# dnjulek/vapoursynth-zip

Measured on AMD Instinct MI355X. Metric: frames/sec at 4K YUV420P16: Bilateral, BoxBlur, SSIMULACRA2 on 1/2/4/8 MI355X, higher is better.
Workload: dtype u16; 1 GPU; vszip.BoxBlur hradius=vradius=13, 3840x2160 YUV420P16, splitmix64 noise, HBM-resident; parallelism=frame-parallel x1, arena_candidates=20

## Files before the change

### vapoursynth-zip_amd/csrc/boxblur_ct.hpp

```cpp
#pragma once
#include <cmath>
#include <cstdlib>
#include <utility>

#include "common.hpp"

namespace {

#ifndef VSZIP_ST_AUX
#define VSZIP_ST_AUX 2
#endif
#ifndef VSZIP_LD_AUX
#define VSZIP_LD_AUX 0
#endif
#ifndef VSZIP_ST8_AUX
#define VSZIP_ST8_AUX 0
#endif
#ifndef VSZIP_ST16_AUX
#define VSZIP_ST16_AUX 2
#endif
constexpr int kStoreAux = VSZIP_ST_AUX, kLoadAux = VSZIP_LD_AUX, kStoreAux8 = VSZIP_ST8_AUX, kStoreAux16 = VSZIP_ST16_AUX;
typedef uint32_t U32x4 __attribute__((ext_vector_type(4)));
typedef uint32_t U32x2 __attribute__((ext_vector_type(2)));

constexpr int kMaxPlanes = 48;
constexpr int PX = 8;

struct BBPlane {
    const void *src;
    void *dst;
    int sstride, dstride;
    int w, h;
    int block0;
    int ntx;
    int nbands;
    int nperiods;
    int cx0;
};

struct BBParams {
    BBPlane p[kMaxPlanes];
    int nplanes;
    int band_rows;
    int nblocks;
};

constexpr int kRingMaxPlanes = 192;
constexpr int kRingMaxBlocks = 8192;
struct RingParams {
    BBPlane p[kRingMaxPlanes];
    int nplanes;
    int nblocks;
    uint8_t plane_of_block[kRingMaxBlocks];
};

__device__ __forceinline__ int ct_tap_row(int k, int i, int radius, int ih) {
    const int dist_from_bottom = ih - 1 - i;
    if (k < radius) return (i < radius - k) ? min(radius - k - i, ih - 1) : (i - radius + k);
    return (dist_from_bottom < k - radius) ? (i - min(k - radius - dist_from_bottom, i)) : (i - radius + k);
}

template <typename T>
struct Raw8;
template <>
struct Raw8<uint16_t> {
    uint4 q;
};
template <>
struct Raw8<uint8_t> {
    uint2 q;
};

__device__ __forceinline__ void unpack8(const Raw8<uint16_t> &r, uint32_t v[PX]) {
    v[0] = r.q.x & 0xffffu; v[1] = r.q.x >> 16;
    v[2] = r.q.y & 0xffffu; v[3] = r.q.y >> 16;
    v[4] = r.q.z & 0xffffu; v[5] = r.q.z >> 16;
    v[6] = r.q.w & 0xffffu; v[7] = r.q.w >> 16;
}

__device__ __forceinline__ void unpack8(const Raw8<uint8_t> &r, uint32_t v[PX]) {
    v[0] = r.q.x & 0xffu; v[1] = (r.q.x >> 8) & 0xffu; v[2] = (r.q.x >> 16) & 0xffu; v[3] = r.q.x >> 24;
    v[4] = r.q.y & 0xffu; v[5] = (r.q.y >> 8) & 0xffu; v[6] = (r.q.y >> 16) & 0xffu; v[7] = r.q.y >> 24;
}

__device__ __forceinline__ void pack8(const uint32_t v[PX], Raw8<uint16_t> &r) {
    r.q.x = v[0] | (v[1] << 16);
    r.q.y = v[2] | (v[3] << 16);
    r.q.z = v[4] | (v[5] << 16);
    r.q.w = v[6] | (v[7] << 16);
}

__device__ __forceinline__ void pack8(const uint32_t v[PX], Raw8<uint8_t> &r) {
    r.q.x = v[0] | (v[1] << 8) | (v[2] << 16) | (v[3] << 24);
    r.q.y = v[4] | (v[5] << 8) | (v[6] << 16) | (v[7] << 24);
}

template <typename T, int PXN>
struct RawN : Raw8<T> {};
template <>
struct RawN<uint8_t, 16> {
    uint4 q;
};
template <typename T>
__device__ __forceinline__ void unpackN(const RawN<T, 8> &r, uint32_t v[8]) {
    unpack8(static_cast<const Raw8<T> &>(r), v);
}
__device__ __forceinline__ void unpackN(const RawN<uint8_t, 16> &r, uint32_t v[16]) {
    const uint32_t dw[4] = {r.q.x, r.q.y, r.q.z, r.q.w};
#pragma unroll
    for (int k = 0; k < 16; ++k) v[k] = (dw[k >> 2] >> (8 * (k & 3))) & 0xffu;
}

__device__ __forceinline__ int mirror_col(int c, int w) {
    c = c < 0 ? -c - 1 : c;
    c = c >= w ? 2 * w - 1 - c : c;
    return min(max(c, 0), w - 1);
}

template <typename T>
__device__ __forceinline__ Raw8<T> load8(const T *row, int vx0, int w, bool fast) {
    Raw8<T> r;
    if (fast) {
        r.q = *reinterpret_cast<const decltype(r.q) *>(row + vx0);
    } else {
        uint32_t v[PX];
#pragma unroll
        for (int k = 0; k < PX; ++k) v[k] = row[mirror_col(vx0 + k, w)];
        pack8(v, r);
    }
    return r;
}

template <typename T>
__device__ __forceinline__ void store8(T *row, int x0, int w, bool fast, const uint32_t o[PX]);

template <>
__device__ __forceinline__ void store8<uint16_t>(uint16_t *row, int x0, int w, bool fast, const uint32_t o[PX]) {
    if (fast) {
        uint4 q;
        q.x = (o[0] & 0xffffu) | (o[1] << 16);
        q.y = (o[2] & 0xffffu) | (o[3] << 16);
        q.z = (o[4] & 0xffffu) | (o[5] << 16);
        q.w = (o[6] & 0xffffu) | (o[7] << 16);
        *reinterpret_cast<uint4 *>(row + x0) = q;
    } else {
#pragma unroll
        for (int k = 0; k < PX; ++k)
            if (x0 + k < w) row[x0 + k] = (uint16_t)o[k];
    }
}

template <>
__device__ __forceinline__ void store8<uint8_t>(uint8_t *row, int x0, int w, bool fast, const uint32_t o[PX]) {
    if (fast) {
        uint2 q;
        q.x = (o[0] & 0xffu) | ((o[1] & 0xffu) << 8) | ((o[2] & 0xffu) << 16) | (o[3] << 24);
        q.y = (o[4] & 0xffu) | ((o[5] & 0xffu) << 8) | ((o[6] & 0xffu) << 16) | (o[7] << 24);
        *reinterpret_cast<uint2 *>(row + x0) = q;
    } else {
#pragma unroll
        for (int k = 0; k < PX; ++k)
            if (x0 + k < w) row[x0 + k] = (uint8_t)o[k];
    }
}

template <int R>
struct CtGeom {
    static constexpr int K = 2 * R + 1;
    static constexpr int NE = (R + 1 + PX - 1) / PX;
    static constexpr int HL = NE * PX;
    static constexpr int HR = ((R + PX - 1) / PX) * PX;
    static constexpr int OUT_LANES = 64 - NE - HL / PX - HR / PX;
    static constexpr int TWO = OUT_LANES * PX;
};

__device__ __forceinline__ void wave_lds_fence() {
    __builtin_amdgcn_fence(__ATOMIC_RELEASE, "wavefront");
    __builtin_amdgcn_wave_barrier();
    __builtin_amdgcn_fence(__ATOMIC_ACQUIRE, "wavefront");
}

template <typename T, int R, bool DPP>
__global__ __launch_bounds__(64) void boxblur_ct_int_kernel(const BBParams prm) {
    using G = CtGeom<R>;
    constexpr uint32_t K = G::K;
    constexpr uint32_t MAGIC = (uint32_t)(((1ull << 32) + K - 1) / K);
    constexpr uint64_t INV = ((1ull << 32) + R) / K;
    constexpr uint32_t INV2 = (uint32_t)(INV >> 16);
    constexpr uint32_t INVLO = (uint32_t)(INV & 0xffffu);

    __shared__ __attribute__((aligned(16))) uint32_t P[64 * PX];

    int pi = 0;
    const int b = blockIdx.x;
#pragma unroll 1
    for (int i = 1; i < prm.nplanes; ++i)
        if (b >= prm.p[i].block0) pi = i;
    const BBPlane pl = prm.p[pi];
    const int lb = b - pl.block0;
    const int tx = lb % pl.ntx;
    const int by = lb / pl.ntx;
    const int w = pl.w, h = pl.h;
    const int y0 = by * prm.band_rows;
    const int y1 = min(y0 + prm.band_rows, h);
    const T *src = static_cast<const T *>(pl.src);
    T *dst = static_cast<T *>(pl.dst);

    const int lane = threadIdx.x;
    const int X0 = tx * G::TWO;
    const int vx0 = lane < G::NE ? lane * PX : X0 - G::HL + (lane - G::NE) * PX;
    constexpr int VB = sizeof(T) * PX;
    const bool src_al = ((reinterpret_cast<uintptr_t>(src) | (uintptr_t)((size_t)pl.sstride * sizeof(T))) & (VB - 1)) == 0;
    const bool dst_al = ((reinterpret_cast<uintptr_t>(dst) | (uintptr_t)((size_t)pl.dstride * sizeof(T))) & (VB - 1)) == 0;
    const bool in_fast = src_al && vx0 >= 0 && vx0 + PX <= w;
    const bool is_out = lane >= G::NE + G::HL / PX && lane < G::NE + G::HL / PX + G::OUT_LANES && vx0 < w;
    const bool out_fast = dst_al && vx0 + PX <= w;

    uint32_t col[PX];
#pragma unroll
    for (int k = 0; k < PX; ++k) col[k] = 0;
#pragma unroll 1
    for (int k = 0; k < (int)K; ++k) {
        uint32_t v[PX];
        unpack8(load8<T>(src + (size_t)ct_tap_row(k, y0, R, h) * pl.sstride, vx0, w, in_fast), v);
#pragma unroll
        for (int j = 0; j < PX; ++j) col[j] += v[j];
    }

    const int ci = lane * PX;
#pragma unroll 1
    for (int i = y0; i < y1; ++i) {
        Raw8<T> an, sn;
        const bool more = i + 1 < y1;
        if (more) {
            const int n = i + 1;
            const int ar = (n + R < h) ? n + R : n - 1;
            const int sr = (n <= R) ? R - n + 1 : n - R - 1;
            an = load8<T>(src + (size_t)ar * pl.sstride, vx0, w, in_fast);
            sn = load8<T>(src + (size_t)sr * pl.sstride, vx0, w, in_fast);
        }

        uint32_t p[PX];
#pragma unroll
        for (int k = 0; k < PX; ++k) p[k] = __umulhi(col[k] + R, MAGIC);
#pragma unroll
        for (int k = 1; k < PX; ++k) p[k] += p[k - 1];
        const uint32_t incl = DPP ? wave_incl_scan_dpp(p[PX - 1]) : wave_incl_scan_shfl(p[PX - 1]);
        const uint32_t base = incl - p[PX - 1];
#pragma unroll
        for (int k = 0; k < PX; ++k) p[k] += base;
        *reinterpret_cast<uint4 *>(&P[ci]) = make_uint4(p[0], p[1], p[2], p[3]);
        *reinterpret_cast<uint4 *>(&P[ci + 4]) = make_uint4(p[4], p[5], p[6], p[7]);
        wave_lds_fence();

        if (is_out) {
            const uint32_t e0 = P[R] + P[R - 1];
            const uint32_t krow = 32768u + (uint32_t)(((uint64_t)e0 * INVLO) >> 16);
            uint32_t o[PX];
#pragma unroll
            for (int k = 0; k < PX; ++k) {
                const uint32_t e = P[ci + k + R] - P[ci + k - R - 1];
                o[k] = (uint32_t)(((uint64_t)e * INV2 + krow) >> 16);
            }
            store8<T>(dst + (size_t)i * pl.dstride, vx0, w, out_fast, o);
        }
        wave_lds_fence();

        if (more) {
            uint32_t a[PX], sb[PX];
            unpack8(an, a);
            unpack8(sn, sb);
#pragma unroll
            for (int k = 0; k < PX; ++k) col[k] += a[k] - sb[k];
        }
    }
}



template <int R, int SLOT_VGPRS = 4, int PXN = 8, int RV = R>
struct RingGeom {
    static constexpr int K = 2 * RV + 1;
    static constexpr int HL = ((R + 1 + PXN - 1) / PXN) * PXN;
    static constexpr int HR = ((R + PXN - 1) / PXN) * PXN;
#ifdef VSZIP_RING_OUT_LANES
    static constexpr int OUT_LANES = VSZIP_RING_OUT_LANES < 64 - HL / PXN - HR / PXN ? VSZIP_RING_OUT_LANES : 64 - HL / PXN - HR / PXN;
#else
    static constexpr int OUT_LANES = 64 - HL / PXN - HR / PXN;
#endif
    static constexpr int TWO = OUT_LANES * PXN;
    static constexpr int est_vgprs(int d) { return (2 * RV + 1 + d) * SLOT_VGPRS + (PXN == 16 ? 104 : 56); }
    static constexpr int tier(int v) { return v <= 128 ? 4 : (v <= 168 ? 3 : 2); }
    static constexpr int D3 = (2 * RV + 4) % 3 == 0 ? 3 : ((2 * RV + 6) % 3 == 0 ? 5 : 7);
#ifdef VSZIP_RING_D
    static constexpr int D = VSZIP_RING_D | 1;
    static constexpr int KL = (2 * RV + 1 + D) % 3 == 0 ? 3 : 2;
#else
    static constexpr bool SHALLOW = tier(est_vgprs(1)) > tier(est_vgprs(D3));
    static constexpr int D = SHALLOW ? 1 : D3;
    static constexpr int KL = SHALLOW ? 2 : 3;
#endif
    static constexpr int NR = 2 * RV + 1 + D;
#ifdef VSZIP_RING_WPE
    static constexpr int WPE = VSZIP_RING_WPE;
#else
    static constexpr int WPE = (SLOT_VGPRS == 2 && PXN == 8) ? (tier(est_vgprs(D)) > 3 ? 3 : tier(est_vgprs(D))) : tier(est_vgprs(D));
#endif
    static_assert(NR % KL == 0, "K-column ring must divide the period");
    static constexpr uint32_t MAGIC = K > 1 ? (uint32_t)(((1ull << 32) + K - 1) / K) : 0u;
};

template <typename T, int R, bool GENERAL, int PXN = 8, bool HONLY = false>
struct RingWave {
    static_assert(PXN == 8 || (PXN == 16 && sizeof(T) == 1 && !GENERAL), "16 pixels a lane: 8-bit planes, whole 16-pixel groups");
    static constexpr int RV = HONLY ? 0 : R;
    using G = RingGeom<R, (int)(sizeof(T) * PXN / 4), PXN, RV>;
    using RawT = RawN<T, PXN>;
    using Vec = decltype(RawT{}.q);
    static constexpr int NR = G::NR;
    static constexpr uint64_t INV = ((1ull << 32) + R) / (uint64_t)(2 * R + 1);
    static constexpr uint32_t INV2 = (uint32_t)(INV >> 16);

    RawT ring[NR];
    uint32_t col[PXN];
    uint32_t kcol;
    uint32_t kwgt;
    uint32_t kvo;
    uint32_t kn[G::KL], ko[G::KL];
    uint32_t kn_off, ko_off;
    uint32_t kr_prev;
    uint32_t *P;
    const char *srcb;
    char *dstb;
    uint32_t coff;
    uint32_t doff;
    uint32_t next_off;
    uint32_t out_off;
    uint32_t srow, drow;
    int w, h, lane, c0;
    bool rev, ld_ok, is_out, out_full;
    bool plain;
    __amdgpu_buffer_rsrc_t rs, rd;
    uint32_t sdoff;
    uint32_t psel;
    static constexpr uint32_t kOOB = 0xfffffff0u;

    __device__ __forceinline__ RawT fetch_off(uint32_t row_off) const {
        RawT t;
        if constexpr (sizeof(T) * PXN == 16) {
            const auto v = __builtin_amdgcn_raw_buffer_load_b128(rs, coff, row_off, sizeof(T) == 2 ? kLoadAux : 0);
            t.q = make_uint4(v[0], v[1], v[2], v[3]);
        } else {
            const auto v = __builtin_amdgcn_raw_buffer_load_b64(rs, coff, row_off, 0);
            t.q = make_uint2(v[0], v[1]);
        }
        return t;
    }
    __device__ __forceinline__ uint32_t fetch_px(uint32_t row_off) const {
        if constexpr (sizeof(T) == 2)
            return __builtin_amdgcn_raw_buffer_load_b16(rs, kvo, row_off, 0);
        else
            return __builtin_amdgcn_raw_buffer_load_b8(rs, kvo, row_off, 0);
    }
    __device__ __forceinline__ uint32_t krow_now() const {
        constexpr uint32_t INVLO = (uint32_t)(INV & 0xffffu);
        uint32_t v = __umul24(G::K > 1 ? __umulhi(kcol, G::MAGIC) : kcol, kwgt);
        v += (uint32_t)__builtin_amdgcn_update_dpp(0, (int)v, 0x111, 0xf, 0xf, false);
        v += (uint32_t)__builtin_amdgcn_update_dpp(0, (int)v, 0x112, 0xf, 0xf, false);
        v += (uint32_t)__builtin_amdgcn_update_dpp(0, (int)v, 0x114, 0xf, 0xf, false);
        v += (uint32_t)__builtin_amdgcn_update_dpp(0, (int)v, 0x118, 0xf, 0xf, false);
        uint32_t e0;
        if constexpr (R < 16) {
            e0 = (uint32_t)__builtin_amdgcn_readlane((int)v, 15);
        } else {
            v += (uint32_t)__builtin_amdgcn_update_dpp(0, (int)v, 0x142, 0xa, 0xf, false);
            e0 = (uint32_t)__builtin_amdgcn_readlane((int)v, 31);
        }
        return 32768u + (uint32_t)(((uint64_t)e0 * INVLO) >> 16);
    }

    __device__ __forceinline__ void fix_order(RawT &r) const {
        if constexpr (GENERAL) return;
        if constexpr (sizeof(T) * PXN == 16) {
            const uint4 o = r.q;
            r.q.x = __builtin_amdgcn_perm(o.w, o.x, psel);
            r.q.y = __builtin_amdgcn_perm(o.z, o.y, psel);
            r.q.z = __builtin_amdgcn_perm(o.y, o.z, psel);
            r.q.w = __builtin_amdgcn_perm(o.x, o.w, psel);
        } else {
            const uint2 o = r.q;
            r.q.x = __builtin_amdgcn_perm(o.y, o.x, psel);
            r.q.y = __builtin_amdgcn_perm(o.x, o.y, psel);
        }
    }
    __device__ __forceinline__ uint32_t row_off(int v) const {
        const int r = v < 0 ? -v : (v < h ? v : v - RV - 1);
        return (uint32_t)min(r, h - 1) * srow;
    }

    template <int J>
    __device__ __forceinline__ void fill(int y0) {
        ring[J] = fetch_off(row_off(y0 - RV + J));
    }
    template <int J>
    __device__ __forceinline__ void accum() {
        uint32_t v[PXN];
        fix_order(ring[J]);
        unpackN(ring[J], v);
#pragma unroll
        for (int k = 0; k < PXN; ++k) col[k] += v[k];
    }
    template <int... J>
    __device__ __forceinline__ void fill_all(int y0, std::integer_sequence<int, J...>) {
        (fill<(J + G::K) % NR>(y0), ...);
    }
    template <int... J>
    __device__ __forceinline__ void accum_all(std::integer_sequence<int, J...>) {
        (accum<J>(), ...);
    }

    static __device__ __forceinline__ int pidx(int c) { return (c & (PXN - 1)) * 64 + c / PXN; }

    __device__ __forceinline__ void window_sums(const uint32_t *Pb, uint32_t e[PXN]) const {
        if constexpr (!GENERAL) {
#pragma unroll
            for (int k = 0; k < PXN; ++k) {
                const int hi = k + R, lo = k - R - 1;
                const int hi_px = hi & (PXN - 1), hi_ln = hi / PXN;
                const int lo_px = lo & (PXN - 1), lo_ln = (lo - lo_px) / PXN;
                e[k] = Pb[hi_px * 64 + lane + hi_ln] - Pb[lo_px * 64 + lane + lo_ln];
            }
        } else {
            const int off = lane * PXN - c0;
            auto lds = [&](int idx) { return Pb[pidx(min(max(idx, 0), 64 * PXN - 1))]; };
            const uint32_t qw = lds(w - 1 + off);
#pragma unroll
            for (int k = 0; k < PXN; ++k) {
                const int x = c0 + k;
                const int lo = x - R - 1, ml = R - x - 1;
                uint32_t v = lds(min(x + R, w - 1) + off) + qw - lds(min(2 * w - 2 - x - R, w - 1) + off);
                v -= lo >= 0 ? lds(lo + off) : 0u;
                v += ml >= 0 ? lds(ml + off) : 0u;
                e[k] = v;
            }
        }
    }

    __device__ __forceinline__ void emit_row(const uint32_t e[PXN], uint32_t row_off_bytes, uint32_t kr, bool live) const {
        if constexpr (GENERAL) {
            if (!live || !is_out) return;
        }
        uint32_t t[PXN];
#pragma unroll
        for (int k = 0; k < PXN; ++k) t[k] = __umul24(e[k], INV2) + kr;
        if constexpr (!GENERAL) {
#ifdef VSZIP_DIAG_NO_STORE
            const uint32_t vo = (live && lane == 8) ? sdoff : kOOB;
#else
            const uint32_t vo = live ? sdoff : kOOB;
#endif
            if constexpr (sizeof(T) == 2) {
                U32x4 v;
                v.x = __builtin_amdgcn_perm(t[1], t[0], 0x07060302u);
                v.y = __builtin_amdgcn_perm(t[3], t[2], 0x07060302u);
                v.z = __builtin_amdgcn_perm(t[5], t[4], 0x07060302u);
                v.w = __builtin_amdgcn_perm(t[7], t[6], 0x07060302u);
                __builtin_amdgcn_raw_buffer_store_b128(v, rd, vo, row_off_bytes, kStoreAux);
            } else if constexpr (PXN == 16) {
                uint32_t dw[4];
#pragma unroll
                for (int g = 0; g < 4; ++g) {
                    const uint32_t a0 = __builtin_amdgcn_perm(t[4 * g + 1], t[4 * g], 0x0c0c0602u);
                    const uint32_t a1 = __builtin_amdgcn_perm(t[4 * g + 3], t[4 * g + 2], 0x0c0c0602u);
                    dw[g] = a0 | (a1 << 16);
                }
                U32x4 v;
                v.x = dw[0];
                v.y = dw[1];
                v.z = dw[2];
                v.w = dw[3];
                __builtin_amdgcn_raw_buffer_store_b128(v, rd, vo, row_off_bytes, kStoreAux16);
            } else {
                U32x2 v;
                const uint32_t a0 = __builtin_amdgcn_perm(t[1], t[0], 0x0c0c0602u);
                const uint32_t a1 = __builtin_amdgcn_perm(t[3], t[2], 0x0c0c0602u);
                const uint32_t a2 = __builtin_amdgcn_perm(t[5], t[4], 0x0c0c0602u);
                const uint32_t a3 = __builtin_amdgcn_perm(t[7], t[6], 0x0c0c0602u);
                v.x = a0 | (a1 << 16);
                v.y = a2 | (a3 << 16);
                __builtin_amdgcn_raw_buffer_store_b64(v, rd, vo, row_off_bytes, kStoreAux8);
            }
        } else {
            T *q = reinterpret_cast<T *>(dstb + (row_off_bytes + doff));
            if (out_full) {
                if constexpr (sizeof(T) == 2) {
                    uint4 v;
                    v.x = __builtin_amdgcn_perm(t[1], t[0], 0x07060302u);
                    v.y = __builtin_amdgcn_perm(t[3], t[2], 0x07060302u);
                    v.z = __builtin_amdgcn_perm(t[5], t[4], 0x07060302u);
                    v.w = __builtin_amdgcn_perm(t[7], t[6], 0x07060302u);
                    *reinterpret_cast<uint4 *>(q) = v;
                } else {
                    uint2 v;
                    const uint32_t a0 = __builtin_amdgcn_perm(t[1], t[0], 0x0c0c0602u);
                    const uint32_t a1 = __builtin_amdgcn_perm(t[3], t[2], 0x0c0c0602u);
                    const uint32_t a2 = __builtin_amdgcn_perm(t[5], t[4], 0x0c0c0602u);
                    const uint32_t a3 = __builtin_amdgcn_perm(t[7], t[6], 0x0c0c0602u);
                    v.x = a0 | (a1 << 16);
                    v.y = a2 | (a3 << 16);
                    *reinterpret_cast<uint2 *>(q) = v;
                }
            } else {
#pragma unroll
                for (int k = 0; k < PXN; ++k)
                    if (c0 + k < w) q[k] = (T)(t[k] >> 16);
            }
        }
    }

    template <int S>
    __device__ __forceinline__ void step(int i, int y0) {
        uint32_t *Pa = P + (S & 1) * (64 * PXN);
        const uint32_t *Pb = P + ((S & 1) ^ 1) * (64 * PXN);
        __builtin_amdgcn_sched_barrier(0);

        uint32_t e[PXN];
        const bool have_prev = S > 0 || i > y0;
#ifdef VSZIP_DIAG_NO_HORIZONTAL
#pragma unroll
        for (int k = 0; k < PXN; ++k) e[k] = col[k];
#else
        if (!GENERAL || have_prev) window_sums(Pb, e);
#endif

        uint32_t p[PXN];
#pragma unroll
        for (int k = 0; k < PXN; ++k) {
            if constexpr (G::K == 1) {
                p[k] = col[k];
            } else if constexpr (sizeof(T) == 1) {
                constexpr uint32_t M19 = (uint32_t)(((1u << 19) + G::K - 1) / G::K);
                static_assert((uint64_t)(255u * G::K + RV) * (M19 * G::K - (1u << 19)) < (1u << 19), "8-bit divide-by-k shortcut must be exact");
                p[k] = __umul24(col[k], M19) >> 19;
            } else {
                p[k] = __umulhi(col[k], G::MAGIC);
            }
        }
        if constexpr (GENERAL) {
            const uint32_t m = ld_ok ? 0xffffffffu : 0u;
#pragma unroll
            for (int k = 0; k < PXN; ++k) p[k] &= m;
        }
#ifdef VSZIP_DIAG_NO_HORIZONTAL
        (void)Pa;
        kr_prev += p[0] + p[7];
#else
#pragma unroll
        for (int k = 1; k < PXN; ++k) p[k] += p[k - 1];
        const uint32_t incl = wave_incl_scan_dpp(p[PXN - 1]);
        const uint32_t base = incl - p[PXN - 1];
#pragma unroll
        for (int k = 0; k < PXN; ++k) Pa[k * 64 + lane] = p[k] + base;
#endif

        {
            constexpr int E = (S + 1 + 2 * RV) % NR;
            uint32_t a[PXN], sb[PXN];
            fix_order(ring[E]);
            unpackN(ring[E], a);
            unpackN(ring[S], sb);
#pragma unroll
            for (int k = 0; k < PXN; ++k) col[k] += a[k] - sb[k];
#ifdef VSZIP_DIAG_NO_LOAD
            if (next_off == 0xffffffffu) ring[S] = fetch_off(next_off);
#else
            ring[S] = fetch_off(next_off);
#endif

        }
        const uint32_t kr_cur = krow_now();
        {
            constexpr int J = S % G::KL;
            kcol += kn[J] - ko[J];
#ifndef VSZIP_DIAG_NO_KCOL
            kn[J] = fetch_px(kn_off);
            ko[J] = fetch_px(ko_off);
#endif

        }

        emit_row(e, out_off, kr_prev, have_prev);
        out_off += have_prev ? drow : 0u;
        kr_prev = kr_cur;
        if (plain) {
            next_off += srow;
            kn_off += srow;
            ko_off += srow;
        } else {
            next_off = row_off(i + 2 + RV + G::D);
            kn_off = row_off(i + 2 + RV + G::KL);
            ko_off = row_off(i + 1 - RV + G::KL);
        }
#ifndef VSZIP_DIAG_NO_FENCE
        wave_lds_fence();
#endif
    }

    template <int... S>
    __device__ __forceinline__ void period(int i0, int y0, std::integer_sequence<int, S...>) {
        (step<S>(i0 + S, y0), ...);
    }
};

template <typename T, int R, bool GENERAL, int PXN = 8, bool HONLY = false>
__global__ __launch_bounds__(64, (GENERAL ? 2 : RingGeom<R, (int)(sizeof(T) * PXN / 4), PXN, (HONLY ? 0 : R)>::WPE)) void boxblur_ct_ring_kernel(const RingParams prm) {
    using W = RingWave<T, R, GENERAL, PXN, HONLY>;
    using G = typename W::G;
    constexpr int RV = W::RV;
    static_assert(G::NR % 2 == 0 && G::NR <= 64, "ring period must be even and fit a wave");
    __shared__ __attribute__((aligned(16))) uint32_t P[2 * 64 * PXN];

    const int chunk = (prm.nblocks + 7) >> 3;
    const int b = (int)(blockIdx.x & 7) * chunk + (int)(blockIdx.x >> 3);
    if (b >= prm.nblocks) return;
    const int pi = prm.plane_of_block[b];
    const BBPlane pl = prm.p[pi];
    const int lb = b - pl.block0;
    const int tx = lb % pl.ntx;
    const int by = lb / pl.ntx;
    const int p0 = (int)((long)by * pl.nperiods / pl.nbands);
    const int p1 = (int)((long)(by + 1) * pl.nperiods / pl.nbands);
    const int band_rows = (p1 - p0) * G::NR;
    const int y0 = min(p0 * G::NR, pl.h - band_rows);
    const int w = pl.w;

    W st;
    st.P = P;
    st.w = w;
    st.h = pl.h;
    st.srow = (uint32_t)pl.sstride * (uint32_t)sizeof(T);
    st.drow = (uint32_t)pl.dstride * (uint32_t)sizeof(T);
    st.srcb = static_cast<const char *>(pl.src);
    st.dstb = static_cast<char *>(pl.dst);
    const int lane = threadIdx.x;
    st.lane = lane;
    const int vc0 = pl.cx0 + tx * G::TWO - G::HL + lane * PXN;
    st.c0 = vc0;
    st.is_out = lane >= G::HL / PXN && lane < G::HL / PXN + G::OUT_LANES && vc0 < w;
    st.doff = (uint32_t)(max(vc0, 0) * (int)sizeof(T));
    st.out_full = vc0 + PXN <= w;
    if constexpr (!GENERAL) {
        int g = vc0;
        st.rev = false;
        if (vc0 < 0) {
            g = -vc0 - PXN;
            st.rev = true;
        } else if (vc0 >= w) {
            g = 2 * w - vc0 - PXN;
            st.rev = true;
        }
        g = min(max(g, 0), w - PXN);
        st.coff = (uint32_t)(g * (int)sizeof(T));
        st.ld_ok = true;
    } else {
        st.rev = false;
        st.ld_ok = vc0 >= 0 && vc0 < w;
        st.coff = (uint32_t)(min(max(vc0, 0), ((w - 1) / PXN) * PXN) * (int)sizeof(T));
    }

    st.psel = st.rev ? (sizeof(T) == 2 ? 0x05040706u : 0x04050607u) : 0x03020100u;
    st.sdoff = st.is_out ? st.doff : W::kOOB;
    st.rs = __builtin_amdgcn_make_buffer_rsrc(const_cast<void *>(pl.src), 0, (int)((uint32_t)pl.h * st.srow), 0x00020000);
    st.rd = __builtin_amdgcn_make_buffer_rsrc(pl.dst, 0, (int)((uint32_t)pl.h * st.drow), 0x00020000);
    st.plain = (y0 - RV >= 0) && (y0 + band_rows + RV + G::D + 2 < pl.h);

    st.fill_all(y0, std::make_integer_sequence<int, G::NR>{});
#pragma unroll
    for (int k = 0; k < PXN; ++k) st.col[k] = RV;
    st.accum_all(std::make_integer_sequence<int, (int)G::K>{});
    {
        const int kc = min(lane, R);
        st.kvo = (uint32_t)(kc * (int)sizeof(T));
        st.kwgt = lane < R ? 2u : (lane == R ? 1u : 0u);
        uint32_t acc = RV;
#pragma unroll
        for (int k = 0; k < (int)G::K; ++k) acc += st.fetch_px(st.row_off(y0 - RV + k));
        st.kcol = acc;
#pragma unroll
        for (int j = 0; j < G::KL; ++j) {
            st.kn[j] = st.fetch_px(st.row_off(y0 + j + 1 + RV));
            st.ko[j] = st.fetch_px(st.row_off(y0 + j - RV));
        }
        st.kn_off = st.row_off(y0 + G::KL + 1 + RV);
        st.ko_off = st.row_off(y0 + G::KL - RV);
        st.kr_prev = 0;
    }
    st.next_off = st.row_off(y0 + 1 + RV + G::D);
    st.out_off = (uint32_t)y0 * st.drow;

    const int y1 = y0 + band_rows;
#pragma unroll 1
    for (int i0 = y0; i0 < y1; i0 += G::NR) st.period(i0, y0, std::make_integer_sequence<int, G::NR>{});
    {
        uint32_t e[PXN];
        st.window_sums(P + 64 * PXN, e);
        st.emit_row(e, st.out_off, st.kr_prev, true);
    }
}


template <typename T, int R>
int launch_ct_int(vszip_ctx *ctx, const vszip_plane *planes, int nplanes) {
    using G = CtGeom<R>;
    int done = 0;
    while (done < nplanes) {
        BBParams prm;
        const int n = std::min(kMaxPlanes, nplanes - done);
        prm.nplanes = n;
        long total_px = 0;
        for (int i = 0; i < n; ++i) total_px += (long)planes[done + i].w * planes[done + i].h;
        int band = 64;
        while (band > 16 && total_px / ((long)G::TWO * band) < 4096) band >>= 1;
        prm.band_rows = band;
        int blocks = 0;
        for (int i = 0; i < n; ++i) {
            const vszip_plane &s = planes[done + i];
            BBPlane &d = prm.p[i];
            d.src = s.src;
            d.dst = s.dst;
            d.sstride = (int)s.src_stride;
            d.dstride = (int)s.dst_stride;
            d.w = s.w;
            d.h = s.h;
            d.block0 = blocks;
            d.ntx = (s.w + G::TWO - 1) / G::TWO;
            d.nbands = (s.h + band - 1) / band;
            blocks += d.ntx * d.nbands;
        }
        if (ctx->scan_mode == 1)
            hipLaunchKernelGGL((boxblur_ct_int_kernel<T, R, false>), dim3(blocks), dim3(64), 0, ctx->stream, prm);
        else
            hipLaunchKernelGGL((boxblur_ct_int_kernel<T, R, true>), dim3(blocks), dim3(64), 0, ctx->stream, prm);
        VSZIP_HIP_CHECK(ctx, hipGetLastError());
        done += n;
    }
    return VSZIP_OK;
}

struct RingSpan {
    int cx0, ntx;
};

template <typename T, int R, int PXN, bool HONLY = false>
int ring_plan(const vszip_plane *planes, const RingSpan *spans, int n, double *waves_ret) {
    using G = typename RingWave<T, R, false, PXN, HONLY>::G;
    struct Geo {
        int h, ntx, count;
    };
    std::vector<Geo> geos;
    for (int i = 0; i < n; ++i) {
        bool found = false;
        for (Geo &g : geos)
            if (g.h == planes[i].h && g.ntx == spans[i].ntx) {
                ++g.count;
                found = true;
                break;
            }
        if (!found) geos.push_back({planes[i].h, spans[i].ntx, 1});
    }
        auto bands_for = [](int h, int P, int target) { return std::max((h % G::NR != 0 && P >= 2) ? 2 : 1, (P + target / 2) / target); };
        const double halo_p = (double)(G::K - 1 + G::D) / G::NR;
        const double slots = 256.0 * 4 * G::WPE;
        double waves_out = 0;
        auto cost_for = [&](int target) {
            double work = 0, waves = 0, max_len = 0;
            for (const Geo &g : geos) {
                const int P = (g.h + G::NR - 1) / G::NR;
                const int nb = bands_for(g.h, P, target);
                const double ntx = (double)g.ntx * g.count;
                work += ntx * (P + nb * halo_p);
                waves += ntx * nb;
                max_len = std::max(max_len, (double)((P + nb - 1) / nb) + halo_p);
            }
            waves_out = waves;
            const double gens = std::ceil(waves / slots);
            const double eff = std::min(1.0, work / (slots * gens * max_len));
            return std::max(work / slots * (1.0 + 0.3 * (1.0 - eff)), 0.3 * max_len);
        };
        int target = 1;
        double best = cost_for(1);
        const double min_waves = std::min(0.6 * slots, waves_out);
        for (int t = 2; t <= 96; ++t) {
            const double c = cost_for(t);
            if (waves_out >= min_waves && c < best) {
                best = c;
                target = t;
            }
        }
        *waves_ret = (cost_for(target), waves_out);
        return target;
}


template <typename T, int R, int PXN, bool GEN, bool HONLY = false>
int launch_ct_ring_spans(vszip_ctx *ctx, const vszip_plane *all_planes, const RingSpan *all_spans, int nall) {
    using G = typename RingWave<T, R, false, PXN, HONLY>::G;
    std::vector<vszip_plane> planes_v;
    std::vector<RingSpan> spans_v;
    for (int i = 0; i < nall; ++i)
        if (all_spans[i].ntx > 0) {
            planes_v.push_back(all_planes[i]);
            spans_v.push_back(all_spans[i]);
        }
    const vszip_plane *planes = planes_v.data();
    const RingSpan *spans = spans_v.data();
    const int nplanes = (int)planes_v.size();
    int done = 0;
    while (done < nplanes) {
        RingParams prm;
        const int n = std::min(kRingMaxPlanes, nplanes - done);
        auto bands_for = [](int h, int P, int target) { return std::max((h % G::NR != 0 && P >= 2) ? 2 : 1, (P + target / 2) / target); };
        double waves_out = 0;
        int target = ring_plan<T, R, PXN, HONLY>(planes + done, spans + done, n, &waves_out);
        if (ctx->opt.ring_periods > 0) target = ctx->opt.ring_periods;
#ifdef VSZIP_RING_PERIODS_FIXED
        target = VSZIP_RING_PERIODS_FIXED;
#endif
#ifdef VSZIP_RING_PLAN_DEBUG
        fprintf(stderr, "ring plan PX%d GEN%d r=%d: n=%d target=%d waves=%.0f slots=%d NR=%d | plane0 %dx%d ntx=%d\n", PXN, (int)GEN, R, n, target, waves_out, 256 * 4 * G::WPE, G::NR,
                planes[done].w, planes[done].h, spans[done].ntx);
#endif
        VSZIP_HIP_CHECK(ctx, hipSetDevice(ctx->device));
        int blocks = 0, fit = n;
        for (int i = 0; i < n; ++i) {
            const vszip_plane &s = planes[done + i];
            BBPlane &d = prm.p[i];
            d.src = s.src;
            d.dst = s.dst;
            d.sstride = (int)s.src_stride;
            d.dstride = (int)s.dst_stride;
            d.w = s.w;
            d.h = s.h;
            d.nperiods = (s.h + G::NR - 1) / G::NR;
            d.nbands = bands_for(s.h, d.nperiods, target);
            d.ntx = spans[done + i].ntx;
            d.cx0 = spans[done + i].cx0;
            d.block0 = blocks;
            if (blocks + d.ntx * d.nbands > kRingMaxBlocks) {
                if (i == 0) return vszip_set_error(ctx, VSZIP_ERR_ARG, "BoxBlur: launch table overflow (%d blocks)", blocks + d.ntx * d.nbands);
                fit = i;
                break;
            }
            for (int k = 0; k < d.ntx * d.nbands; ++k) prm.plane_of_block[blocks + k] = (uint8_t)i;
            blocks += d.ntx * d.nbands;
        }
        prm.nplanes = fit;
        prm.nblocks = blocks;
        const dim3 grid(((blocks + 7) / 8) * 8);
        {
            vszip_probe_scope probe(ctx);
            hipLaunchKernelGGL((boxblur_ct_ring_kernel<T, R, GEN, PXN, HONLY>), grid, dim3(64), 0, ctx->stream, prm);
        }
        VSZIP_HIP_CHECK(ctx, hipGetLastError());
        done += fit;
    }
    return VSZIP_OK;
}

template <typename T>
bool ring_ok(const vszip_plane *planes, int nplanes) {
    constexpr uintptr_t VB = sizeof(T) * PX;
    for (int i = 0; i < nplanes; ++i) {
        const vszip_plane &p = planes[i];
        if ((reinterpret_cast<uintptr_t>(p.src) | reinterpret_cast<uintptr_t>(p.dst) | (uintptr_t)(p.src_stride * sizeof(T)) | (uintptr_t)(p.dst_stride * sizeof(T))) & (VB - 1)) return false;
        if (p.src_stride < ((p.w + PX - 1) / PX) * PX) return false;
        if (p.src_stride < 24) return false;
        if (p.h < 2 * 22 + 1 + 8) return false;
        if ((uint64_t)p.src_stride * p.h * sizeof(T) >= (1ull << 32) || (uint64_t)p.dst_stride * p.h * sizeof(T) >= (1ull << 32)) return false;
    }
    return true;
}

constexpr int kRing16MaxR = 19;
template <typename T, int R, bool HONLY = false>
bool ring16_ok(const vszip_ctx *ctx, const vszip_plane *planes, int nplanes) {
    if (sizeof(T) != 1 || ctx->opt.ct_u8_px8) return false;
    using G16 = RingGeom<R, 4, 16, (HONLY ? 0 : R)>;
    using G8 = RingGeom<R, 2, 8, (HONLY ? 0 : R)>;
    double px = 0, t16 = 0, t8 = 0;
    for (int i = 0; i < nplanes; ++i) {
        const vszip_plane &p = planes[i];
        if (p.w < 32) return false;
        if ((reinterpret_cast<uintptr_t>(p.src) | reinterpret_cast<uintptr_t>(p.dst) | (uintptr_t)p.src_stride | (uintptr_t)p.dst_stride) & 15) return false;
        px += (double)p.w * p.h;
        t16 += (double)((p.w + G16::TWO - 1) / G16::TWO) * G16::TWO * p.h;
        t8 += (double)((p.w + G8::TWO - 1) / G8::TWO) * G8::TWO * p.h;
    }
    if (R >= 8 && px / t16 < 0.93 * (px / t8)) return false;
    if (R >= 8) {
        const int n = std::min(nplanes, kRingMaxPlanes);
        std::vector<RingSpan> s16(n), s8(n);
        for (int i = 0; i < n; ++i) {
            s16[i] = {0, (planes[i].w + G16::TWO - 1) / G16::TWO};
            s8[i] = {0, (planes[i].w + G8::TWO - 1) / G8::TWO};
        }
        double w16 = 0, w8 = 0;
        ring_plan<T, R, 16, HONLY>(planes, s16.data(), n, &w16);
        ring_plan<T, R, 8, HONLY>(planes, s8.data(), n, &w8);
        const double f16 = w16 / (256.0 * 4 * G16::WPE), f8 = w8 / (256.0 * 4 * G8::WPE);
        if (f16 < 0.8 && f8 > f16 + 0.05) return false;
    }
    return true;
}

template <typename T, int R, int PXF, bool HONLY = false>
int run_ct_ring(vszip_ctx *ctx, const vszip_plane *planes, int nplanes) {
    using GF = typename RingWave<T, R, false, PXF, HONLY>::G;
    using GG = typename RingWave<T, R, true, 8, HONLY>::G;
    std::vector<RingSpan> fast(nplanes), rest(nplanes);
    bool any_rest = false, any_fast = false;
    for (int i = 0; i < nplanes; ++i) {
        const int w = planes[i].w;
        if (w % PXF == 0) {
            fast[i] = {0, (w + GF::TWO - 1) / GF::TWO};
            rest[i] = {0, 0};
        } else {
            const int room = w + GF::HL - 64 * PXF;
            const int nsafe = room >= 0 ? room / GF::TWO + 1 : 0;
            fast[i] = {0, nsafe};
            const int x = nsafe * GF::TWO;
            rest[i] = {x, (w - x + GG::TWO - 1) / GG::TWO};
        }
        any_fast = any_fast || fast[i].ntx > 0;
        any_rest = any_rest || rest[i].ntx > 0;
    }
    if (any_fast) {
        const int rc = launch_ct_ring_spans<T, R, PXF, false, HONLY>(ctx, planes, fast.data(), nplanes);
        if (rc != VSZIP_OK) return rc;
    }
    if (any_rest) return launch_ct_ring_spans<T, R, 8, true, HONLY>(ctx, planes, rest.data(), nplanes);
    return VSZIP_OK;
}

#ifdef VSZIP_DEV_R
#define VSZIP_R_ENABLED(R) ((R) == VSZIP_DEV_R)
#else
#define VSZIP_R_ENABLED(R) true
#endif

template <typename T, int R, int RLO>
struct CtIntDispatch {
    static int run(vszip_ctx *ctx, int r, const vszip_plane *planes, int nplanes) {
        if constexpr (VSZIP_R_ENABLED(R)) if (r == R) {
            if (ctx->scan_mode == 0 && ring_ok<T>(planes, nplanes)) {
                if constexpr (sizeof(T) == 1 && R <= kRing16MaxR) {
                    if (ring16_ok<T, R>(ctx, planes, nplanes)) return run_ct_ring<T, R, 16>(ctx, planes, nplanes);
                }
                return run_ct_ring<T, R, 8>(ctx, planes, nplanes);
            }
            return launch_ct_int<T, R>(ctx, planes, nplanes);
        }
        if constexpr (R > RLO)
            return CtIntDispatch<T, R - 1, RLO>::run(ctx, r, planes, nplanes);
        else
            return vszip_set_error(ctx, VSZIP_ERR_ARG, "BoxBlur: CT radius not built (development build?)");
    }
    static int run_h(vszip_ctx *ctx, int r, const vszip_plane *planes, int nplanes) {
        if constexpr (VSZIP_R_ENABLED(R)) if (r == R) {
            if (ctx->scan_mode != 0 || !ring_ok<T>(planes, nplanes)) return VSZIP_ERR_UNSUPPORTED;
            if constexpr (sizeof(T) == 1) {
                if (ring16_ok<T, R, true>(ctx, planes, nplanes)) return run_ct_ring<T, R, 16, true>(ctx, planes, nplanes);
            }
            return run_ct_ring<T, R, 8, true>(ctx, planes, nplanes);
        }
        if constexpr (R > RLO)
            return CtIntDispatch<T, R - 1, RLO>::run_h(ctx, r, planes, nplanes);
        else
            return VSZIP_ERR_UNSUPPORTED;
    }
};

}
```

Baseline: 112,400 frames/s.

## Split ring bands by exact row counts and alternate sweep direction per band

Bands are now split on exact row boundaries instead of whole ring periods, and a partial final period runs through a guarded tail. Before, bands were aligned to periods and clamped, so neighbouring bands overlapped and recomputed rows. Alternate bands sweep bottom-up with negative strides, likely so that adjacent bands touch their shared halo rows at about the same time and get cache reuse. The cost is more complex addressing (a direction multiply in the non-plain path), a tail unroll, and a changed band-count heuristic.

```diff
diff --git a/vapoursynth-zip_amd/csrc/boxblur_ct.hpp b/vapoursynth-zip_amd/csrc/boxblur_ct.hpp
--- a/vapoursynth-zip_amd/csrc/boxblur_ct.hpp
+++ b/vapoursynth-zip_amd/csrc/boxblur_ct.hpp
@@ -34,7 +34,6 @@
     int block0;
     int ntx;
     int nbands;
-    int nperiods;
     int cx0;
 };
 
@@ -338,6 +337,8 @@
     uint32_t out_off;
     uint32_t srow, drow;
     int w, h, lane, c0;
+    int ystart, dir;
+    uint32_t sstep, dstep;
     bool rev, ld_ok, is_out, out_full;
     bool plain;
     __amdgpu_buffer_rsrc_t rs, rd;
@@ -399,8 +400,8 @@
     }
 
     template <int J>
-    __device__ __forceinline__ void fill(int y0) {
-        ring[J] = fetch_off(row_off(y0 - RV + J));
+    __device__ __forceinline__ void fill() {
+        ring[J] = fetch_off(row_off(ystart + dir * (J - RV)));
     }
     template <int J>
     __device__ __forceinline__ void accum() {
@@ -411,8 +412,8 @@
         for (int k = 0; k < PXN; ++k) col[k] += v[k];
     }
     template <int... J>
-    __device__ __forceinline__ void fill_all(int y0, std::integer_sequence<int, J...>) {
-        (fill<(J + G::K) % NR>(y0), ...);
+    __device__ __forceinline__ void fill_all(std::integer_sequence<int, J...>) {
+        (fill<(J + G::K) % NR>(), ...);
     }
     template <int... J>
     __device__ __forceinline__ void accum_all(std::integer_sequence<int, J...>) {
@@ -519,13 +520,13 @@
     }
 
     template <int S>
-    __device__ __forceinline__ void step(int i, int y0) {
+    __device__ __forceinline__ void step(int t) {
         uint32_t *Pa = P + (S & 1) * (64 * PXN);
         const uint32_t *Pb = P + ((S & 1) ^ 1) * (64 * PXN);
         __builtin_amdgcn_sched_barrier(0);
 
         uint32_t e[PXN];
-        const bool have_prev = S > 0 || i > y0;
+        const bool have_prev = S > 0 || t > 0;
 #ifdef VSZIP_DIAG_NO_HORIZONTAL
 #pragma unroll
         for (int k = 0; k < PXN; ++k) e[k] = col[k];
@@ -590,16 +591,16 @@
         }
 
         emit_row(e, out_off, kr_prev, have_prev);
-        out_off += have_prev ? drow : 0u;
+        out_off += have_prev ? dstep : 0u;
         kr_prev = kr_cur;
         if (plain) {
-            next_off += srow;
-            kn_off += srow;
-            ko_off += srow;
+            next_off += sstep;
+            kn_off += sstep;
+            ko_off += sstep;
         } else {
-            next_off = row_off(i + 2 + RV + G::D);
-            kn_off = row_off(i + 2 + RV + G::KL);
-            ko_off = row_off(i + 1 - RV + G::KL);
+            next_off = row_off(ystart + dir * (t + 2 + RV + G::D));
+            kn_off = row_off(ystart + dir * (t + 2 + RV + G::KL));
+            ko_off = row_off(ystart + dir * (t + 1 - RV + G::KL));
         }
 #ifndef VSZIP_DIAG_NO_FENCE
         wave_lds_fence();
@@ -607,8 +608,12 @@
     }
 
     template <int... S>
-    __device__ __forceinline__ void period(int i0, int y0, std::integer_sequence<int, S...>) {
-        (step<S>(i0 + S, y0), ...);
+    __device__ __forceinline__ void period(int t0, std::integer_sequence<int, S...>) {
+        (step<S>(t0 + S), ...);
+    }
+    template <int... S>
+    __device__ __forceinline__ void tail(int t0, int n, std::integer_sequence<int, S...>) {
+        (void)((t0 + S < n ? (step<S>(t0 + S), true) : false) && ...);
     }
 };
 
@@ -628,10 +633,9 @@
     const int lb = b - pl.block0;
     const int tx = lb % pl.ntx;
     const int by = lb / pl.ntx;
-    const int p0 = (int)((long)by * pl.nperiods / pl.nbands);
-    const int p1 = (int)((long)(by + 1) * pl.nperiods / pl.nbands);
-    const int band_rows = (p1 - p0) * G::NR;
-    const int y0 = min(p0 * G::NR, pl.h - band_rows);
+    const int y0 = (int)((long)by * pl.h / pl.nbands);
+    const int y1 = (int)((long)(by + 1) * pl.h / pl.nbands);
+    const bool up = !HONLY && ((by + pi) & 1) != 0;
     const int w = pl.w;
 
     W st;
@@ -672,11 +676,16 @@
     st.sdoff = st.is_out ? st.doff : W::kOOB;
     st.rs = __builtin_amdgcn_make_buffer_rsrc(const_cast<void *>(pl.src), 0, (int)((uint32_t)pl.h * st.srow), 0x00020000);
     st.rd = __builtin_amdgcn_make_buffer_rsrc(pl.dst, 0, (int)((uint32_t)pl.h * st.drow), 0x00020000);
-    st.plain = (y0 - RV >= 0) && (y0 + band_rows + RV + G::D + 2 < pl.h);
-
-    st.fill_all(y0, std::make_integer_sequence<int, G::NR>{});
+    st.dir = up ? -1 : 1;
+    st.ystart = up ? y1 - 1 : y0;
+    st.sstep = up ? 0u - st.srow : st.srow;
+    st.dstep = up ? 0u - st.drow : st.drow;
+    constexpr int AHEAD = 2 + (G::D > G::KL ? G::D : G::KL);
+    st.plain = up ? (y0 - RV - AHEAD >= 0) && (y1 + RV <= pl.h) : (y0 - RV >= 0) && (y1 + RV + G::D + 2 < pl.h);
+
 #pragma unroll
     for (int k = 0; k < PXN; ++k) st.col[k] = RV;
+    st.fill_all(std::make_integer_sequence<int, G::NR>{});
     st.accum_all(std::make_integer_sequence<int, (int)G::K>{});
     {
         const int kc = min(lane, R);
@@ -684,26 +693,28 @@
         st.kwgt = lane < R ? 2u : (lane == R ? 1u : 0u);
         uint32_t acc = RV;
 #pragma unroll
-        for (int k = 0; k < (int)G::K; ++k) acc += st.fetch_px(st.row_off(y0 - RV + k));
+        for (int k = 0; k < (int)G::K; ++k) acc += st.fetch_px(st.row_off(st.ystart - RV + k));
         st.kcol = acc;
 #pragma unroll
         for (int j = 0; j < G::KL; ++j) {
-            st.kn[j] = st.fetch_px(st.row_off(y0 + j + 1 + RV));
-            st.ko[j] = st.fetch_px(st.row_off(y0 + j - RV));
-        }
-        st.kn_off = st.row_off(y0 + G::KL + 1 + RV);
-        st.ko_off = st.row_off(y0 + G::KL - RV);
+            st.kn[j] = st.fetch_px(st.row_off(st.ystart + st.dir * (j + 1 + RV)));
+            st.ko[j] = st.fetch_px(st.row_off(st.ystart + st.dir * (j - RV)));
+        }
+        st.kn_off = st.row_off(st.ystart + st.dir * (G::KL + 1 + RV));
+        st.ko_off = st.row_off(st.ystart + st.dir * (G::KL - RV));
         st.kr_prev = 0;
     }
-    st.next_off = st.row_off(y0 + 1 + RV + G::D);
-    st.out_off = (uint32_t)y0 * st.drow;
-
-    const int y1 = y0 + band_rows;
+    st.next_off = st.row_off(st.ystart + st.dir * (1 + RV + G::D));
+    st.out_off = (uint32_t)st.ystart * st.drow;
+
+    const int n = y1 - y0;
+    const int nfull = n - n % G::NR;
 #pragma unroll 1
-    for (int i0 = y0; i0 < y1; i0 += G::NR) st.period(i0, y0, std::make_integer_sequence<int, G::NR>{});
+    for (int t0 = 0; t0 < nfull; t0 += G::NR) st.period(t0, std::make_integer_sequence<int, G::NR>{});
+    if (nfull < n) st.tail(nfull, n, std::make_integer_sequence<int, G::NR>{});
     {
         uint32_t e[PXN];
-        st.window_sums(P + 64 * PXN, e);
+        st.window_sums(P + ((n - 1) & 1) * (64 * PXN), e);
         st.emit_row(e, st.out_off, st.kr_prev, true);
     }
 }
@@ -751,6 +762,8 @@
     int cx0, ntx;
 };
 
+inline int ring_bands_for(int h, int nr, int target) { return std::max(1, (h + target * nr / 2) / (target * nr)); }
+
 template <typename T, int R, int PXN, bool HONLY = false>
 int ring_plan(const vszip_plane *planes, const RingSpan *spans, int n, double *waves_ret) {
     using G = typename RingWave<T, R, false, PXN, HONLY>::G;
@@ -768,19 +781,17 @@
             }
         if (!found) geos.push_back({planes[i].h, spans[i].ntx, 1});
     }
-        auto bands_for = [](int h, int P, int target) { return std::max((h % G::NR != 0 && P >= 2) ? 2 : 1, (P + target / 2) / target); };
         const double halo_p = (double)(G::K - 1 + G::D) / G::NR;
         const double slots = 256.0 * 4 * G::WPE;
         double waves_out = 0;
         auto cost_for = [&](int target) {
             double work = 0, waves = 0, max_len = 0;
             for (const Geo &g : geos) {
-                const int P = (g.h + G::NR - 1) / G::NR;
-                const int nb = bands_for(g.h, P, target);
+                const int nb = ring_bands_for(g.h, G::NR, target);
                 const double ntx = (double)g.ntx * g.count;
-                work += ntx * (P + nb * halo_p);
                 waves += ntx * nb;
-                max_len = std::max(max_len, (double)((P + nb - 1) / nb) + halo_p);
+                work += ntx * ((double)g.h / G::NR + nb * halo_p);
+                max_len = std::max(max_len, (double)((g.h + nb - 1) / nb) / G::NR + halo_p);
             }
             waves_out = waves;
             const double gens = std::ceil(waves / slots);
@@ -819,7 +830,6 @@
     while (done < nplanes) {
         RingParams prm;
         const int n = std::min(kRingMaxPlanes, nplanes - done);
-        auto bands_for = [](int h, int P, int target) { return std::max((h % G::NR != 0 && P >= 2) ? 2 : 1, (P + target / 2) / target); };
         double waves_out = 0;
         int target = ring_plan<T, R, PXN, HONLY>(planes + done, spans + done, n, &waves_out);
         if (ctx->opt.ring_periods > 0) target = ctx->opt.ring_periods;
@@ -841,8 +851,7 @@
             d.dstride = (int)s.dst_stride;
             d.w = s.w;
             d.h = s.h;
-            d.nperiods = (s.h + G::NR - 1) / G::NR;
-            d.nbands = bands_for(s.h, d.nperiods, target);
+            d.nbands = ring_bands_for(s.h, G::NR, target);
             d.ntx = spans[done + i].ntx;
             d.cx0 = spans[done + i].cx0;
             d.block0 = blocks;
```

Result: faster. 115,300 frames/s (median of 6 runs) (+2.6%).
